# AmbiqAI/nnsp

Hardware: NVIDIA B200
Metric: audio-sec/sec (16 kHz streams, VAD+KWS+S2I cascade) (higher is better)
Workload: dtype int16 activations x int8 weights, int32/int64 accumulate (bit-exact integer path)

## Files before the change

### nnsp_b200/csrc/nnsp_engine.cu

```cuda
#include <cuda_runtime.h>
#include <mutex>
#include <new>
#include <stdlib.h>
#include <string.h>

#include "nnsp_feat.cuh"
#include "nnsp_host.h"
#include "nnsp_net.cuh"
#include "nnsp_tma.cuh"

namespace nnsp {

std::atomic<long long> g_launches{0}, g_tc5_launches{0};
std::atomic<long long> g_cascade_net_launches[3] = {};

static std::mutex g_mu;
static DevTables *g_dev_tables[64] = { nullptr };
static int g_sm_count[64] = { 0 };

int select_device(int device)
{
    int n = 0;
    cudaError_t e = cudaGetDeviceCount(&n);
    if (e != cudaSuccess || n <= 0) {
        nnsp_set_error("no CUDA device available (%s); nnsp-b200 has no CPU fallback", cudaGetErrorString(e));
        return NNSP_B200_ERR_CUDA;
    }
    if (device < 0 || device >= n || device >= 64) { nnsp_set_error("device %d out of range (have %d)", device, n); return NNSP_B200_ERR_ARG; }
    NNSP_CUDA(cudaSetDevice(device));
    std::lock_guard<std::mutex> lk(g_mu);
    if (!g_sm_count[device]) {
        cudaDeviceProp p;
        NNSP_CUDA(cudaGetDeviceProperties(&p, device));
        if (p.major < 10) {
            nnsp_set_error("device %d is sm_%d%d; this library is built for sm_100a only", device, p.major, p.minor);
            return NNSP_B200_ERR_CUDA;
        }
        g_sm_count[device] = p.multiProcessorCount;
    }
    return NNSP_B200_OK;
}
int sm_count(int device) { return g_sm_count[device] ? g_sm_count[device] : 148; }

static bool fill_dev_tables(const nnsp_tables *t, DevTables *d)
{
    bool ok = true;
    memset(d, 0, sizeof *d);
    for (int p = 0; p < 240; p++) d->win2[p] = make_int2((int)t->stft_win[2 * p], (int)t->stft_win[2 * p + 1]);
    auto unpack = [](int32_t w) { return make_int2((int)(int16_t)(w & 0xffff), (int)(w >> 16)); };
    for (int a = 0; a < 4; a++)
        for (int n = 0; n < 3; n++)
            for (int L = 0; L < 16; L++) d->tw0[a][n][L] = unpack(t->fft_tw[4 * (L + 16 * a) + 1 + n]);
    for (int n = 0; n < 3; n++)
        for (int L = 0; L < 16; L++) d->tw1[n][L] = unpack(t->fft_tw[16 * L + 1 + n]);
    for (int m = 0; m < 4; m++)
        for (int n = 0; n < 3; n++) d->tw2[m][n] = unpack(t->fft_tw[64 * m + 1 + n]);
    {
        auto one = [](int2 w) { return w.x == 0x7fff && w.y == 0; };
        auto diag = [](int2 w) { return w.x == w.y; };
        auto adiag = [](int2 w) { return w.y == -(w.x + 1); };
        if (!(one(d->tw2[0][0]) && one(d->tw2[0][1]) && one(d->tw2[0][2]) && adiag(d->tw2[1][0]) &&
              d->tw2[2][0].x == 0 && d->tw2[2][0].y == -32768 && adiag(d->tw2[2][1]) && diag(d->tw2[2][2]) && diag(d->tw2[3][0])))
            ok = false;
    }
    for (int k = 0; k < 256; k++) d->rtw[k] = unpack(t->rfft_tw[k]);
    d->rtw[256] = make_int2(0, 0);
    {
        int g = 0;
        for (int b = 0; b < 40; b++) {
            const int s0 = t->mel_start[b], e0 = t->mel_end[b], bin0 = s0 & ~3, ng = ((e0 | 3) - bin0 + 1) / 4;
            d->mel_meta[b] = (uint32_t)g | ((uint32_t)ng << 8) | ((uint32_t)bin0 << 16);
            if (ng > (b >= 24 ? MEL_MAXG0 : (b >= 8 ? MEL_MAXG1 : MEL_MAXG2)) || g + ng > MEL_GROUPS) ok = false;
            for (int i = 0; i < ng; i++, g++) {
                int w[4];
                for (int k = 0; k < 4; k++) {
                    const int bin = bin0 + 4 * i + k;
                    w[k] = (bin >= s0 && bin <= e0) ? (int)t->mel_taps[t->mel_off[b] + bin - s0] : 0;
                }
                if (g < MEL_GROUPS) d->mel_tap4[g] = make_int4(w[0], w[1], w[2], w[3]);
            }
        }
    }
    memcpy(d->log_lut, t->log_lut, sizeof d->log_lut);
    memcpy(d->tanh_lut, t->tanh_lut, sizeof d->tanh_lut);
    auto tanh_def = [&](int64_t xi) -> int64_t {
        if (xi >= (5 << 15)) return 0x7fff;
        int64_t kx = (xi - 512) >> 10;
        kx = kx < 0 ? 0 : kx;
        const int64_t v = (int64_t)t->tanh_lut[2 * kx] + (((xi - 512 - (kx << 10)) * (int64_t)t->tanh_lut[2 * kx + 1]) >> 15);
        return v > 0 ? v : 0;
    };
    for (int w = 0; w < 320; w++) {
        const int64_t k = w >= 1 ? (w - 1) >> 1 : 0, s = t->tanh_lut[2 * k + 1];
        int64_t lo = INT64_MIN, hi = INT64_MAX;
        for (int64_t dd = 0; dd < 512; dd++) {
            const int64_t y = tanh_def(512 * w + dd);
            lo = std::max(lo, y * 32768 - dd * s);
            hi = std::min(hi, (y + 1) * 32768 - dd * s);
        }
        if (lo >= hi || lo < 0 || lo + 511 * s > INT32_MAX) ok = false;
        d->tanh2[w] = make_int2((int)s, (int)lo);
    }
    d->tanh2[320] = make_int2(0, 0x7fff << 15);
    for (int64_t xi = 0; xi < (5 << 15) + 2048 && ok; xi++) {
        const int64_t w = std::min<int64_t>(xi >> 9, 320), dd = xi - (w << 9);
        if (((dd * d->tanh2[w].x + d->tanh2[w].y) >> 15) != tanh_def(xi)) ok = false;
    }
    return ok;
}

int get_device_tables(int device, const DevTables **out)
{
    std::lock_guard<std::mutex> lk(g_mu);
    if (!g_dev_tables[device]) {
        const nnsp_tables *t = nnsp_tables_get();
        if (!t) { nnsp_set_error("constant-table self check failed (fingerprint mismatch)"); return NNSP_B200_ERR_ARG; }
        DevTables h;
        if (!fill_dev_tables(t, &h)) { nnsp_set_error("constant tables do not have the structure the kernels compile in (mel group bounds, stage-2 twiddles, folded tanh table)"); return NNSP_B200_ERR_ARG; }
        DevTables *d = nullptr;
        NNSP_CUDA(cudaMalloc(&d, sizeof h));
        NNSP_CUDA(cudaMemcpy(d, &h, sizeof h, cudaMemcpyHostToDevice));
        NNSP_CUDA(cudaDeviceSynchronize());
        g_dev_tables[device] = d;
    }
    *out = g_dev_tables[device];
    return NNSP_B200_OK;
}

static void pack_matrix(uint32_t *dst, const int8_t *w, int nrows, int nrows_pad, int cols, int k4)
{
    for (int k = 0; k < k4; k++)
        for (int r = 0; r < nrows_pad; r++) {
            uint32_t word = 0;
            for (int b = 0; b < 4; b++) {
                const int c = 4 * k + b;
                const uint8_t v = (r < nrows && c < cols) ? (uint8_t)w[(size_t)r * cols + c] : 0;
                word |= (uint32_t)v << (8 * b);
            }
            dst[(size_t)k * nrows_pad + r] = word;
        }
}

int upload_model(const nnsp_b200_model *m, DeviceModel *out)
{
    DevModel &D = out->h;
    memset(&D, 0, sizeof D);
    D.nn_id = m->nn_id;
    D.numlayers = m->numlayers;
    D.n_out = m->size_layer[m->numlayers];
    D.feat_rshift = 30 - m->layer[0].qi;
    memcpy(D.mean, m->mean, sizeof D.mean);
    memcpy(D.stdR, m->stdR, sizeof D.stdR);
    for (int i = 0; i < 40; i++) {
        int64_t t = ((int64_t)-147963 - (int64_t)m->mean[i]) * (int64_t)m->stdR[i];
        t >>= D.feat_rshift;
        t = t > 32767 ? 32767 : (t < -32768 ? -32768 : t);
        D.silence[i] = (int16_t)t;
    }
    int woff = 0, boff = 0;
    for (int i = 0; i < m->numlayers; i++) {
        const nnsp_layer &L = m->layer[i];
        DevLayer &G = D.layer[i];
        G.type = L.type; G.act = L.act; G.rows = L.rows; G.cols = L.cols; G.acc32 = L.acc32;
        G.nrows = (L.type == NNSP_LAYER_LSTM) ? 4 * L.rows : L.rows;
        G.nrows_pad = (G.nrows + 31) & ~31;
        G.k4 = (L.cols + 3) / 4;
        G.k4rec = (L.type == NNSP_LAYER_LSTM) ? (L.rows + 3) / 4 : 0;
        const int qi_out = (L.type == NNSP_LAYER_LSTM) ? L.qi_next : L.qi;
        const int qs = (qi_out + L.qk) > 15 ? (qi_out + L.qk) : 15;
        G.sh_x = (L.type == NNSP_LAYER_LSTM) ? (L.qi_next - L.qi) : 0;
        G.sh_bias = qs - L.qb;
// ... 6 lines not shown
        if (L.cols > 480) { nnsp_set_error("layer %d: %d inputs exceed the exact-int32 dot-product bound (480)", i, L.cols); return NNSP_B200_ERR_UNSUPPORTED; }
    }
    if (D.h_stride > NNSP_B200_MAX_WIDTH) { nnsp_set_error("total LSTM state %d exceeds %d", D.h_stride, NNSP_B200_MAX_WIDTH); return NNSP_B200_ERR_UNSUPPORTED; }
    D.weight_words = (woff + 3) & ~3;
    D.bias_count = (boff + 7) & ~7;
    uint32_t *hw = (uint32_t *)calloc((size_t)D.weight_words + 4, 4);
    int16_t *hb = (int16_t *)calloc((size_t)D.bias_count + 8, 2);
    if (!hw || !hb) { free(hw); free(hb); return NNSP_B200_ERR_NOMEM; }
    for (int i = 0; i < m->numlayers; i++) {
        const nnsp_layer &L = m->layer[i];
        const DevLayer &G = D.layer[i];
        pack_matrix(hw + G.w_off, L.w, G.nrows, G.nrows_pad, L.cols, G.k4);
        if (L.type == NNSP_LAYER_LSTM) pack_matrix(hw + G.wrec_off, L.wrec, G.nrows, G.nrows_pad, L.rows, G.k4rec);
        memcpy(hb + G.bias_off, L.bias, (size_t)G.nrows * 2);
    }
    cudaError_t e1 = cudaMalloc(&out->wimg, (size_t)D.weight_words * 4);
    cudaError_t e2 = cudaMalloc(&out->bimg, (size_t)D.bias_count * 2);
    cudaError_t e3 = cudaMalloc(&out->d, sizeof D);
    if (e1 == cudaSuccess && e2 == cudaSuccess && e3 == cudaSuccess) {
        e1 = cudaMemcpy(out->wimg, hw, (size_t)D.weight_words * 4, cudaMemcpyHostToDevice);
        e2 = cudaMemcpy(out->bimg, hb, (size_t)D.bias_count * 2, cudaMemcpyHostToDevice);
        e3 = cudaMemcpy(out->d, &D, sizeof D, cudaMemcpyHostToDevice);
    }
    free(hw);
    free(hb);
    if (e1 != cudaSuccess || e2 != cudaSuccess || e3 != cudaSuccess) {
        nnsp_set_error("model upload failed: %s", cudaGetErrorString(e1 != cudaSuccess ? e1 : (e2 != cudaSuccess ? e2 : e3)));
        free_model(out);
        return NNSP_B200_ERR_CUDA;
    }
    return NNSP_B200_OK;
}

void free_model(DeviceModel *dm)
{
    if (dm->wimg) cudaFree(dm->wimg);
    if (dm->bimg) cudaFree(dm->bimg);
    if (dm->d) cudaFree(dm->d);
    dm->wimg = nullptr; dm->bimg = nullptr; dm->d = nullptr;
}

#ifndef FEAT_WARPS_PER_CTA
#define FEAT_WARPS_PER_CTA 8
#endif
constexpr int FEAT_WARPS = FEAT_WARPS_PER_CTA;
constexpr int FEAT_THREADS = FEAT_WARPS * 32;
#ifndef FEAT_CTAS_PER_SM
#define FEAT_CTAS_PER_SM 3
#endif
#ifndef FEAT_ITERS
#define FEAT_ITERS 8
#endif

struct FeatSmem {
    FeatSmemTables tb;
    FrameScratch fs[FEAT_WARPS * 2];
    int32_t norm[84];
};

template <bool RAGGED>
__global__ void __launch_bounds__(FEAT_THREADS, FEAT_CTAS_PER_SM)
feat_kernel(const DevTables *__restrict__ tables, const int16_t *__restrict__ pcm, long long stride,
            const int16_t *__restrict__ hist, int hist_frames, int s0, int ns, int T,
            int32_t *__restrict__ logmel, const int32_t *__restrict__ norm, int16_t *__restrict__ feat16,
            const int32_t *__restrict__ nfr)
{
    extern __shared__ __align__(128) unsigned char smem_raw[];
    FeatSmem &sm = *reinterpret_cast<FeatSmem *>(smem_raw);
    load_feat_tables(&sm.tb, tables, threadIdx.x, FEAT_THREADS);
    if (norm && threadIdx.x < 81) sm.norm[threadIdx.x] = norm[threadIdx.x];
    const int32_t *snorm = norm ? sm.norm : nullptr;
    __syncthreads();
    const int warp = threadIdx.x >> 5, lane = threadIdx.x & 31, half = lane >> 4, L = lane & 15;
    FrameScratch &fs = sm.fs[warp * 2 + half];
    const long long F = (long long)ns * T;
    const int hist_len = hist_frames * NNSP_B200_FRAME;
    for (long long f0 = ((long long)blockIdx.x * FEAT_WARPS + warp) * 2; f0 < F; f0 += (long long)gridDim.x * FEAT_WARPS * 2) {
        const long long f = f0 + half;
        bool valid = f < F;
        const long long fc = valid ? f : 0;
        const int s = s0 + (int)(fc / T), t = (int)(fc % T);
        if (RAGGED) {
            valid = valid && t < stream_frames(nfr, s, T);
            if (!__any_sync(0xffffffffu, valid)) continue;
        }
        const int base = (t - 2) * NNSP_B200_FRAME;
        const unsigned int *pw = reinterpret_cast<const unsigned int *>(pcm + (long long)s * stride + base) + L;
        const unsigned int *hw = reinterpret_cast<const unsigned int *>(hist + (long long)s * hist_len + hist_len + base) + L;
        const int pth = (2 - t) * (NNSP_B200_FRAME / 2);
        auto load_pair = [&](int a, int p) -> uint32_t {
            if (RAGGED && !valid) return 0u;
            return (p < pth) ? __ldg(hw + 16 * a) : __ldg(pw + 16 * a);
        };
        const long long row = ((long long)s * T + t) * NNSP_B200_NMEL;
        frame_logmel<false>(sm.tb, fs, L, load_pair, logmel + row, valid, FeatDump{}, snorm, feat16 + row);
    }
}

int launch_feature(const DevTables *tb, const FeatLaunch &a, int device, cudaStream_t st)
{
    static bool attr_set[64] = { false };
    static std::mutex attr_mu;
    std::unique_lock<std::mutex> attr_lk(attr_mu);
    if (!attr_set[device]) {
        NNSP_CUDA(cudaFuncSetAttribute(feat_kernel<false>, cudaFuncAttributeMaxDynamicSharedMemorySize, (int)sizeof(FeatSmem)));
        NNSP_CUDA(cudaFuncSetAttribute(feat_kernel<true>, cudaFuncAttributeMaxDynamicSharedMemorySize, (int)sizeof(FeatSmem)));
        attr_set[device] = true;
    }
    attr_lk.unlock();
    const long long F = (long long)a.ns * a.T;
    if (F <= 0) return NNSP_B200_OK;
    long long blocks = (F + FEAT_WARPS * 2 - 1) / (FEAT_WARPS * 2);
    const long long cap = (long long)sm_count(device) * FEAT_CTAS_PER_SM;
    long long iters = blocks / (cap * 8);
    iters = iters < FEAT_ITERS ? FEAT_ITERS : (iters > 4 * FEAT_ITERS ? 4 * FEAT_ITERS : iters);
    static const int iters_env = [] { const char *e = getenv("NNSP_B200_FEAT_ITERS"); return e ? atoi(e) : 0; }();
    if (iters_env > 0) iters = iters_env;
    const long long chunked = (blocks + iters - 1) / iters;
    if (blocks > cap) blocks = chunked > cap ? ((chunked + cap / 2) / cap) * cap : cap;
    static const int pad = [] { const char *e = getenv("NNSP_B200_FEAT_SMEM_PAD"); return e ? atoi(e) : 0; }();
    if (pad > 0) {
        static bool pad_set[64] = { false };
        if (!pad_set[device]) {
            NNSP_CUDA(cudaFuncSetAttribute(feat_kernel<false>, cudaFuncAttributeMaxDynamicSharedMemorySize, (int)sizeof(FeatSmem) + pad));
            NNSP_CUDA(cudaFuncSetAttribute(feat_kernel<true>, cudaFuncAttributeMaxDynamicSharedMemorySize, (int)sizeof(FeatSmem) + pad));
            pad_set[device] = true;
        }
    }
    const size_t smem = sizeof(FeatSmem) + (pad > 0 ? pad : 0);
    if (a.nfr)
        feat_kernel<true><<<(unsigned)blocks, FEAT_THREADS, smem, st>>>(tb, a.pcm, a.stride, a.hist, a.hist_frames, a.s0, a.ns, a.T,
                                                                       a.logmel, a.norm, a.feat16, a.nfr);
    else
        feat_kernel<false><<<(unsigned)blocks, FEAT_THREADS, smem, st>>>(tb, a.pcm, a.stride, a.hist, a.hist_frames, a.s0, a.ns, a.T,
                                                                        a.logmel, a.norm, a.feat16, nullptr);
    NNSP_LAUNCH_CHECK();
    return NNSP_B200_OK;
}

template <bool RAGGED>
__global__ void hist_kernel(const unsigned int *__restrict__ src, long long stride_words, unsigned int *__restrict__ hist,
                            int hist_frames, int wpf, int s0, int ns, int T_call, const int32_t *__restrict__ nfr)
{
    const int warp = (blockIdx.x * blockDim.x + threadIdx.x) >> 5, lane = threadIdx.x & 31;
    if (warp >= ns) return;
    const int s = s0 + warp;
    const int T = RAGGED ? stream_frames(nfr, s, T_call) : T_call;
    if (RAGGED && T == 0) return;
    const int words = hist_frames * wpf;
    const int keep = hist_frames - T;
// ... 203 lines not shown
        o.x = s0 | (s1 << 16); o.y = s2 | (s3 << 16); o.z = s4 | (s5 << 16); o.w = s6 | (s7 << 16);
        pcm[gidx] = o;
    }
}

int launch_ingest(const uint32_t *raw_dev, int16_t *pcm_dev, long long n_frames, int device, cudaStream_t st)
{
    if (n_frames <= 0) return NNSP_B200_OK;
    const long long groups = n_frames * (NNSP_B200_FRAME / 8);
    long long blocks = (groups + 255) / 256;
    const long long cap = (long long)sm_count(device) * 8;
    if (blocks > cap) blocks = cap;
    ingest_audadc_kernel<<<(unsigned)blocks, 256, 0, st>>>((const uint4 *)raw_dev, (uint4 *)pcm_dev, groups);
    NNSP_LAUNCH_CHECK();
    return NNSP_B200_OK;
}

__global__ void __launch_bounds__(256) int_peak_kernel(int *sink, int iters, int mode)
{
    int a[8], b[8];
    long long w[8];
#pragma unroll
    for (int i = 0; i < 8; i++) { a[i] = threadIdx.x * 7 + i * 13 + blockIdx.x; b[i] = a[i] ^ 0x55; w[i] = a[i]; }
    const int m = (int)threadIdx.x | 1, c = blockIdx.x + 3;
    if (mode == 0) {
        for (int it = 0; it < iters; it++) {
#pragma unroll
            for (int i = 0; i < 8; i++) { a[i] = a[i] * m + c; a[i] = a[i] * c + m; }
        }
    } else if (mode == 1) {
        for (int it = 0; it < iters; it++) {
#pragma unroll
            for (int i = 0; i < 8; i++) { a[i] = a[i] * m + c; b[i] = (b[i] >> 1) ^ it; }
#pragma unroll
            for (int i = 0; i < 8; i++) { a[i] = a[i] * c + m; b[i] = b[i] + (it | c); }
        }
    } else if (mode == 2) {
        for (int it = 0; it < iters; it++) {
#pragma unroll
            for (int i = 0; i < 8; i++) { w[i] += (long long)a[i] * m; w[i] += (long long)b[i] * c; }
        }
    } else {
        for (int it = 0; it < iters; it++) {
#pragma unroll
            for (int i = 0; i < 8; i++) { a[i] = __dp2a_lo(m, c, a[i]); a[i] = __dp2a_hi(c, m, a[i]); }
        }
    }
    int r = 0;
#pragma unroll
    for (int i = 0; i < 8; i++) r ^= a[i] ^ b[i] ^ (int)w[i] ^ (int)(w[i] >> 32);
    if (r == 0x7fffffff) sink[threadIdx.x] = r;
}

__global__ void __launch_bounds__(FEAT_THREADS)
feat_stages_kernel(const DevTables *__restrict__ tables, const int16_t *__restrict__ windows, int n,
                   int32_t *fft_in, int32_t *spec, int32_t *pspec, int32_t *mel, int32_t *logmel)
{
    extern __shared__ __align__(128) unsigned char smem_raw[];
    FeatSmem &sm = *reinterpret_cast<FeatSmem *>(smem_raw);
    load_feat_tables(&sm.tb, tables, threadIdx.x, FEAT_THREADS);
    __syncthreads();
    const int warp = threadIdx.x >> 5, lane = threadIdx.x & 31, half = lane >> 4, L = lane & 15;
    FrameScratch &fs = sm.fs[warp * 2 + half];
    for (int f0 = (blockIdx.x * FEAT_WARPS + warp) * 2; f0 < n; f0 += gridDim.x * FEAT_WARPS * 2) {
        const int f = f0 + half;
        const bool valid = f < n;
        const int fc = valid ? f : 0;
        const int16_t *w = windows + (long long)fc * 480;
        auto load_pair = [&](int a, int p) -> uint32_t { return *reinterpret_cast<const unsigned int *>(w + 2 * p); };
        FeatDump d;
        d.fft_in = fft_in ? fft_in + (long long)fc * 512 : nullptr;
        d.spec = spec ? spec + (long long)fc * 514 : nullptr;
        d.pspec = pspec ? pspec + (long long)fc * 257 : nullptr;
        d.mel = mel ? mel + (long long)fc * 40 : nullptr;
        frame_logmel<true>(sm.tb, fs, L, load_pair, logmel + (long long)fc * 40, valid, d);
    }
}

}

using namespace nnsp;

#define HOST_RING 4

struct nnsp_b200_batch {
    int device = 0, S = 0;
    cudaStream_t stream = nullptr;
    cudaStream_t xs[4] = { nullptr, nullptr, nullptr, nullptr };
    const DevTables *tables = nullptr;
    DeviceModel dm;
    MmaDeviceModel mm;
    bool mma_ok = false, split_ok = false;
    int nn_path = 0;
    int slides = 1;
    uint8_t *sp_planes[2] = { nullptr, nullptr };
    int32_t *sp_dec = nullptr;
    long long sp_cap_inf = 0;
    int16_t *feat16[2] = { nullptr, nullptr }; long long feat16_frames = 0;
    cudaStream_t nn_stream = nullptr;
    cudaEvent_t ev_feat[2] = { nullptr, nullptr }, ev_nn[2] = { nullptr, nullptr }, ev_nn0 = nullptr;
    bool nn_pending[2] = { false, false }, last_piped = false;
    unsigned pipe = 0;
    int32_t *norm_dev = nullptr;
    StreamState st{};
    int16_t thresh_prob = 0, th_count = 0;
    int32_t *logmel = nullptr; long long logmel_frames = 0;
    int16_t *d_pcm = nullptr; long long d_pcm_frames = 0;
    nnsp_b200_result *d_res = nullptr; long long d_res_frames = 0;
    NNSmemLayout lay{};
    int nn_ctas_per_sm = 1;
    cudaEvent_t ev[3] = { nullptr, nullptr, nullptr };
    bool ev_valid = false;
// ... 476 lines not shown
        NE_CUDA(cudaMemcpy(b->feat16[0], row5, N * 40 * sizeof(int16_t), cudaMemcpyHostToDevice));
        NE_CUDA(cudaDeviceSynchronize());
        NNLaunch l{};
        l.tables = b->tables; l.st = b->st; l.s0 = 0; l.ns = n; l.T = 1; l.taps = tp;
        l.thresh_prob = b->thresh_prob; l.th_count = b->th_count;
        if ((rc = launch_nn_split(b->mm, l, b->feat16[0], 0, 1, b->sp_planes[0], b->sp_planes[1], b->sp_dec, (int)b->sp_cap_inf, b->device, b->stream))) return done(rc);
    } else {
        NE_CUDA(cudaMemcpy(b->st.ctx, x, N * 240 * sizeof(int16_t), cudaMemcpyHostToDevice));
        NE_CUDA(cudaDeviceSynchronize());
        if (path == 2) {
            NNLaunch l{};
            l.tables = b->tables; l.st = b->st; l.s0 = 0; l.ns = n; l.T = 1; l.taps = tp; l.raw_ctx = 1;
            l.thresh_prob = b->thresh_prob; l.th_count = b->th_count;
            if ((rc = launch_nn_mma(b->mm, l, b->device, b->stream))) return done(rc);
        } else {
            NNArgs a{};
            a.model = b->dm.d; a.wimg = b->dm.wimg; a.bimg = b->dm.bimg; a.tables = b->tables; a.st = b->st;
            a.s0 = 0; a.ns = n; a.T = 1; a.taps = tp; a.raw_ctx = 1;
            a.thresh_prob = b->thresh_prob; a.th_count = b->th_count;
            int blocks = (n + NN_WARPS - 1) / NN_WARPS;
            const int cap = sm_count(b->device) * b->nn_ctas_per_sm;
            if (blocks > cap) blocks = cap;
            nn_kernel<<<blocks, NN_THREADS, b->lay.total, b->stream>>>(a, (int)b->lay.b, (int)b->lay.lut, (int)b->lay.model, (int)b->lay.scratch);
            g_launches.fetch_add(1);
            NE_CUDA(cudaGetLastError());
        }
    }
    NE_CUDA(cudaStreamSynchronize(b->stream));
    if (act && D.act_stride > 0) NE_CUDA(cudaMemcpy(act, t_act, N * D.act_stride * sizeof(int16_t), cudaMemcpyDeviceToHost));
    if (logits) NE_CUDA(cudaMemcpy(logits, t_logits, N * NO * sizeof(int32_t), cudaMemcpyDeviceToHost));
    if (h1 && HS > 0) NE_CUDA(cudaMemcpy(h1, t_h, N * HS * sizeof(int16_t), cudaMemcpyDeviceToHost));
    if (c1 && HS > 0) NE_CUDA(cudaMemcpy(c1, t_c, N * HS * sizeof(int32_t), cudaMemcpyDeviceToHost));
#undef NE_CUDA
    return done(NNSP_B200_OK);
}


int nnsp_b200_feature_stages(int device, const int16_t *windows, int n, int32_t *fft_in, int32_t *spec,
                             int32_t *pspec, int32_t *mel, int32_t *logmel)
{
    if (!windows || n <= 0) return NNSP_B200_ERR_ARG;
    int rc = select_device(device);
    if (rc) return rc;
    const DevTables *tb;
    if ((rc = get_device_tables(device, &tb))) return rc;
    int16_t *dw = nullptr;
    int32_t *dbuf = nullptr;
    const size_t per = 512 + 514 + 257 + 40 + 40;
    NNSP_CUDA(cudaMalloc(&dw, (size_t)n * 480 * 2));
    NNSP_CUDA(cudaMalloc(&dbuf, (size_t)n * per * 4));
    NNSP_CUDA(cudaMemcpy(dw, windows, (size_t)n * 480 * 2, cudaMemcpyHostToDevice));
    NNSP_CUDA(cudaDeviceSynchronize());
    int32_t *d_fi = dbuf, *d_sp = d_fi + (size_t)n * 512, *d_ps = d_sp + (size_t)n * 514, *d_me = d_ps + (size_t)n * 257, *d_lm = d_me + (size_t)n * 40;
    NNSP_CUDA(cudaFuncSetAttribute(feat_stages_kernel, cudaFuncAttributeMaxDynamicSharedMemorySize, (int)sizeof(FeatSmem)));
    int blocks = (n + FEAT_WARPS * 2 - 1) / (FEAT_WARPS * 2);
    if (blocks > 1024) blocks = 1024;
    feat_stages_kernel<<<blocks, FEAT_THREADS, sizeof(FeatSmem)>>>(tb, dw, n, d_fi, d_sp, d_ps, d_me, d_lm);
    NNSP_LAUNCH_CHECK();
    NNSP_CUDA(cudaDeviceSynchronize());
    if (fft_in) NNSP_CUDA(cudaMemcpy(fft_in, d_fi, (size_t)n * 512 * 4, cudaMemcpyDeviceToHost));
    if (spec) NNSP_CUDA(cudaMemcpy(spec, d_sp, (size_t)n * 514 * 4, cudaMemcpyDeviceToHost));
    if (pspec) NNSP_CUDA(cudaMemcpy(pspec, d_ps, (size_t)n * 257 * 4, cudaMemcpyDeviceToHost));
    if (mel) NNSP_CUDA(cudaMemcpy(mel, d_me, (size_t)n * 40 * 4, cudaMemcpyDeviceToHost));
    if (logmel) NNSP_CUDA(cudaMemcpy(logmel, d_lm, (size_t)n * 40 * 4, cudaMemcpyDeviceToHost));
    cudaFree(dw);
    cudaFree(dbuf);
    return NNSP_B200_OK;
}

int nnsp_b200_ingest_audadc(int device, const uint32_t *raw_dev, int16_t *pcm_dev, long long n_frames, void *stream)
{
    if (!raw_dev || !pcm_dev || n_frames < 0 || ((uintptr_t)raw_dev & 15) || ((uintptr_t)pcm_dev & 15)) {
        nnsp_set_error("ingest: null or not 16-byte aligned buffers");
        return NNSP_B200_ERR_ARG;
    }
    int rc = select_device(device);
    if (rc) return rc;
    return launch_ingest(raw_dev, pcm_dev, n_frames, device, (cudaStream_t)stream);
}

int nnsp_b200_table(const char *name, const void **data, int *elem_bytes)
{
    const nnsp_tables *t = nnsp_tables_get();
    if (!t || !name || !data || !elem_bytes) return NNSP_B200_ERR_ARG;
    struct { const char *n; const void *p; int eb, cnt; } tab[] = {
        { "stft_win", t->stft_win, 2, 480 }, { "fft_tw", t->fft_tw, 4, 256 }, { "rfft_tw", t->rfft_tw, 4, 256 },
        { "bitrev", t->bitrev, 2, 256 }, { "mel", t->mel, 2, 534 }, { "log_lut", t->log_lut, 2, 256 },
        { "tanh_lut", t->tanh_lut, 2, 384 },
    };
    for (auto &e : tab)
        if (!strcmp(e.n, name)) { *data = e.p; *elem_bytes = e.eb; return e.cnt; }
    return NNSP_B200_ERR_ARG;
}

int nnsp_b200_event_create(int device, void **event)
{
    int rc = select_device(device);
    if (rc) return rc;
    cudaEvent_t e;
    NNSP_CUDA(cudaEventCreate(&e));
    *event = (void *)e;
    return NNSP_B200_OK;
}
int nnsp_b200_event_record(void *event, void *stream) { NNSP_CUDA(cudaEventRecord((cudaEvent_t)event, (cudaStream_t)stream)); return NNSP_B200_OK; }
int nnsp_b200_event_elapsed_ms(void *start, void *stop, float *ms)
{
    NNSP_CUDA(cudaEventSynchronize((cudaEvent_t)stop));
    NNSP_CUDA(cudaEventElapsedTime(ms, (cudaEvent_t)start, (cudaEvent_t)stop));
    return NNSP_B200_OK;
}
// ... 59 lines not shown
```

### nnsp_b200/csrc/nnsp_engine.cuh

```cuda
#pragma once
#include <stdint.h>
#include "nnsp_b200.h"

namespace nnsp {

constexpr int MEL_GROUPS = 144;
constexpr int MEL_MAXG0 = 8, MEL_MAXG1 = 4, MEL_MAXG2 = 2;

struct DevTables {
    int4     mel_tap4[MEL_GROUPS];
    int2     win2[240];
    int2     tw0[4][3][16];
    int2     tw1[3][16];
    int2     tw2[4][3];
    int2     rtw[257];
    uint32_t mel_meta[40];
    int16_t  log_lut[256];
    int16_t  tanh_lut[384];
    int2     tanh2[321];
};

struct DevLayer {
    int type, act;
    int rows;
    int nrows;
    int nrows_pad;
    int cols, k4;
    int k4rec;
    int acc32;
    int sh_x;
    int sh_bias;
    int sh_out;
    int w_off, wrec_off;
    int bias_off;
};

struct DevModel {
    int      nn_id, numlayers;
    int      act_stride, h_stride, n_out;
    int      feat_rshift;
    int      weight_words, bias_count;
    int32_t  mean[40], stdR[40];
    int16_t  silence[40];
    DevLayer layer[NNSP_B200_MAX_LAYERS];
};

enum { SC_TRIGGER = 0, SC_OUT0 = 1, SC_CNT0 = 4, SC_ARGMAX_LAST = 12, SC_SLIDES = 13, SC_RAN = 14, SC_STAGE = 15, SC_N = 16 };

enum { CS_POS = 0, CS_CNT_KWS = 1, CS_CNT_S2I = 2, CS_AGE = 3, CS_N = 4 };

struct StreamState {
    int16_t *ctx;
    int16_t *h;
    int32_t *c;
    int16_t *scal;
    int16_t *hist;
    int32_t *lmhist;
    uint16_t *casc;
};

}
```

### nnsp_b200/csrc/nnsp_feat.cuh

```cuda
#pragma once
#include "nnsp_device.cuh"
#include "nnsp_engine.cuh"

namespace nnsp {

struct FeatSmemTables {
    int4     mel_tap4[MEL_GROUPS];
    int2     win2[240];
    int2     tw0[4][3][16];
    int2     tw1[3][16];
    int2     tw2[4][3];
    int2     rtw[257];
    uint32_t mel_meta[40];
    int16_t  log_lut[256];
};

struct alignas(16) FrameScratch {
    int2    x[272];
};

struct FeatDump {
    int32_t *fft_in, *spec, *pspec, *mel;
};

// ... 15 lines not shown
{
    const int32_t s1r = cr + dr, s1i = ci + di, d1r = cr - dr, d1i = ci - di;
    const int32_t o0r = add3(ar, br, s1r), o0i = add3(ai, bi, s1i);
    const int32_t o1r = add2sub(ar, br, s1r), o1i = add2sub(ai, bi, s1i);
    const int32_t o2r = sub2add(ar, br, d1i), o2i = sub3(ai, bi, d1r);
    const int32_t o3r = sub3(ar, br, d1i), o3i = sub2add(ai, bi, d1r);
    ar = mul_one_q15(o0r);
    ai = mul_one_q15(o0i);
    if (ALLONE) {
        cr = mul_one_q15(o1r); ci = mul_one_q15(o1i);
        br = mul_one_q15(o2r); bi = mul_one_q15(o2i);
        dr = mul_one_q15(o3r); di = mul_one_q15(o3i);
    } else {
        const int32_t w1r = w1.x, w1i = w1.y, w2r = w2.x, w2i = w2.y, w3r = w3.x, w3i = w3.y;
        cr = msub_q15(o1r, w1r, o1i, w1i); ci = madd_q15(o1r, w1i, o1i, w1r);
        br = msub_q15(o2r, w2r, o2i, w2i); bi = madd_q15(o2r, w2i, o2i, w2r);
        dr = msub_q15(o3r, w3r, o3i, w3i); di = madd_q15(o3r, w3i, o3i, w3r);
    }
}

enum { TW_ANY = 0, TW_ONE = 1, TW_NEGI = 2, TW_DIAG = 3, TW_ADIAG = 4 };
template <int KIND>
__device__ __forceinline__ void cmul_tw(int32_t or_, int32_t oi, int2 w, int32_t &re, int32_t &im)
{
    if (KIND == TW_ONE) { re = mul_one_q15(or_); im = mul_one_q15(oi); }
    else if (KIND == TW_NEGI) { re = oi; im = -or_; }
    else if (KIND == TW_DIAG) {
        re = (int32_t)(((int64_t)(or_ - oi) * (int64_t)w.x) >> 15);
        im = (int32_t)(((int64_t)(or_ + oi) * (int64_t)w.x) >> 15);
    } else if (KIND == TW_ADIAG) {
        re = (int32_t)(((int64_t)(or_ + oi) * (int64_t)w.x + (int64_t)oi) >> 15);
        im = (int32_t)(((int64_t)(oi - or_) * (int64_t)w.x - (int64_t)or_) >> 15);
    } else { re = msub_q15(or_, w.x, oi, w.y); im = madd_q15(or_, w.y, oi, w.x); }
}
template <int K1, int K2, int K3>
__device__ __forceinline__ void bfly4_tw(int32_t &ar, int32_t &ai, int32_t &cr, int32_t &ci,
                                         int32_t &br, int32_t &bi, int32_t &dr, int32_t &di,
                                         int2 w1, int2 w2, int2 w3)
{
    const int32_t s1r = cr + dr, s1i = ci + di, d1r = cr - dr, d1i = ci - di;
    const int32_t o0r = add3(ar, br, s1r), o0i = add3(ai, bi, s1i);
    const int32_t o1r = add2sub(ar, br, s1r), o1i = add2sub(ai, bi, s1i);
    const int32_t o2r = sub2add(ar, br, d1i), o2i = sub3(ai, bi, d1r);
    const int32_t o3r = sub3(ar, br, d1i), o3i = sub2add(ai, bi, d1r);
    ar = mul_one_q15(o0r);
    ai = mul_one_q15(o0i);
    cmul_tw<K1>(o1r, o1i, w1, cr, ci);
    cmul_tw<K2>(o2r, o2i, w2, br, bi);
    cmul_tw<K3>(o3r, o3i, w3, dr, di);
}

__device__ __forceinline__ int xpad(int p) { return p + (p >> 4); }

template <bool DUMP, typename LoadPair>
__device__ __forceinline__ void frame_logmel(const FeatSmemTables &tb, FrameScratch &fs, int L,
                                             LoadPair load_pair, int32_t *__restrict__ out_logmel,
                                             bool store, FeatDump dump, const int32_t *norm = nullptr,
                                             int16_t *__restrict__ out_feat = nullptr)
{
    int32_t xr[16], xi[16];
#pragma unroll
    for (int a = 0; a < 15; a++) {
        const int p = L + 16 * a;
        const uint32_t s = load_pair(a, p);
        const int2 w = tb.win2[p];
        xr[a] = (w.x * (int32_t)(int16_t)(s & 0xffff)) >> 15;
        xi[a] = (w.y * ((int32_t)s >> 16)) >> 15;
    }
    xr[15] = 0; xi[15] = 0;
    if (DUMP && dump.fft_in && store) {
#pragma unroll
        for (int a = 0; a < 16; a++) { dump.fft_in[2 * (L + 16 * a)] = xr[a]; dump.fft_in[2 * (L + 16 * a) + 1] = xi[a]; }
    }
#pragma unroll
    for (int a = 0; a < 4; a++) {
        bfly4<false>(xr[a], xi[a], xr[a + 4], xi[a + 4], xr[a + 8], xi[a + 8], xr[a + 12], xi[a + 12],
                     tb.tw0[a][0][L], tb.tw0[a][1][L], tb.tw0[a][2][L]);
    }
    {
        const int2 w1 = tb.tw1[0][L], w2 = tb.tw1[1][L], w3 = tb.tw1[2][L];
#pragma unroll
        for (int g = 0; g < 4; g++)
            bfly4<false>(xr[4 * g], xi[4 * g], xr[4 * g + 1], xi[4 * g + 1], xr[4 * g + 2], xi[4 * g + 2],
                         xr[4 * g + 3], xi[4 * g + 3], w1, w2, w3);
    }
#pragma unroll
    for (int a = 0; a < 16; a++) fs.x[xpad(L + 16 * a)] = make_int2(xr[a], xi[a]);
    __syncwarp();
#pragma unroll
    for (int b = 0; b < 16; b++) { const int2 v = fs.x[xpad(16 * L + b)]; xr[b] = v.x; xi[b] = v.y; }
    __syncwarp();
    bfly4_tw<TW_ONE, TW_ONE, TW_ONE>(xr[0], xi[0], xr[4], xi[4], xr[8], xi[8], xr[12], xi[12], tb.tw2[0][0], tb.tw2[0][1], tb.tw2[0][2]);
    bfly4_tw<TW_ADIAG, TW_ANY, TW_ANY>(xr[1], xi[1], xr[5], xi[5], xr[9], xi[9], xr[13], xi[13], tb.tw2[1][0], tb.tw2[1][1], tb.tw2[1][2]);
    bfly4_tw<TW_NEGI, TW_ADIAG, TW_DIAG>(xr[2], xi[2], xr[6], xi[6], xr[10], xi[10], xr[14], xi[14], tb.tw2[2][0], tb.tw2[2][1], tb.tw2[2][2]);
    bfly4_tw<TW_DIAG, TW_ANY, TW_ANY>(xr[3], xi[3], xr[7], xi[7], xr[11], xi[11], xr[15], xi[15], tb.tw2[3][0], tb.tw2[3][1], tb.tw2[3][2]);
#pragma unroll
    for (int g = 0; g < 4; g++)
        bfly4<true>(xr[4 * g], xi[4 * g], xr[4 * g + 1], xi[4 * g + 1], xr[4 * g + 2], xi[4 * g + 2],
                    xr[4 * g + 3], xi[4 * g + 3], make_int2(0, 0), make_int2(0, 0), make_int2(0, 0));
#pragma unroll
    for (int b = 0; b < 16; b++) {
        const int m = (int)(__brev((unsigned)(16 * L + b)) >> 24);
        fs.x[m] = make_int2(xr[b], xi[b]);
    }
    __syncwarp();
    int32_t pa[8], pb[8];
    int32_t p0 = 0, p256 = 0;
#pragma unroll
    for (int j = 0; j < 8; j++) {
        const bool centre = (j == 0 && L == 0);
        const int i = centre ? 128 : L + 16 * j;
        const int2 zi = fs.x[i], zr = fs.x[256 - i];
        const int2 w = tb.rtw[i], v = tb.rtw[256 - i];
        const int32_t er = (zi.x + zr.x) >> 1, ei = (zi.y - zr.y) >> 1;
        const int32_t orr = (zi.y + zr.y) >> 1, oi = (zr.x - zi.x) >> 1;
        const int32_t xr0 = er + msub_q15(orr, w.x, oi, w.y), xi0 = ei + madd_q15(orr, w.y, oi, w.x);
        pa[j] = (int32_t)(((int64_t)xr0 * xr0 + (int64_t)xi0 * xi0) >> 15);
        const int32_t fi = (zr.y - zi.y) >> 1, pi = (zi.x - zr.x) >> 1;
        const int32_t xr1 = er + msub_q15(orr, v.x, pi, v.y), xi1 = fi + madd_q15(orr, v.y, pi, v.x);
        pb[j] = (int32_t)(((int64_t)xr1 * xr1 + (int64_t)xi1 * xi1) >> 15);
        if (DUMP && dump.spec && store) {
            dump.spec[2 * i] = xr0; dump.spec[2 * i + 1] = xi0;
            if (!centre) { dump.spec[2 * (256 - i)] = xr1; dump.spec[2 * (256 - i) + 1] = xi1; }
        }
    }
    if (DUMP && L == 0) {
        const int2 z0 = fs.x[0], w = tb.rtw[0];
        const int32_t er = z0.x, orr = z0.y;
        const int32_t xr0 = er + msub_q15(orr, w.x, 0, w.y), xi0 = madd_q15(orr, w.y, 0, w.x);
        const int32_t re = z0.x - z0.y;
        p0 = (int32_t)(((int64_t)xr0 * xr0 + (int64_t)xi0 * xi0) >> 15);
        p256 = (int32_t)(((int64_t)re * re) >> 15);
        if (dump.spec && store) { dump.spec[0] = xr0; dump.spec[1] = xi0; dump.spec[512] = re; dump.spec[513] = 0; }
    }
    __syncwarp();
    int32_t *ps = reinterpret_cast<int32_t *>(fs.x);
#pragma unroll
    for (int j = 0; j < 8; j++) {
        const bool centre = (j == 0 && L == 0);
        const int i = centre ? 128 : L + 16 * j;
        ps[i] = pa[j];
        if (!centre) ps[256 - i] = pb[j];
    }
    if (DUMP && L == 0) { ps[0] = p0; ps[256] = p256; }
    __syncwarp();
    if (DUMP && dump.pspec && store)
        for (int i = L; i < 257; i += 16) dump.pspec[i] = ps[i];
#pragma unroll
    for (int r = 0; r < 3; r++) {
        const int b = 39 - L - 16 * r;
        if (b >= 0) {
            const uint32_t meta = tb.mel_meta[b];
            const int ng = (meta >> 8) & 0xff;
            const int4 *tap = &tb.mel_tap4[meta & 0xff];
            const int4 *bin = reinterpret_cast<const int4 *>(&ps[meta >> 16]);
            int64_t m0 = 0, m1 = 0;
#pragma unroll
            for (int i = 0; i < (r == 0 ? MEL_MAXG0 : (r == 1 ? MEL_MAXG1 : MEL_MAXG2)); i++) {
                if (i < ng) {
                    const int4 w = tap[i], v = bin[i];
                    m0 += (int64_t)w.x * (int64_t)v.x; m1 += (int64_t)w.y * (int64_t)v.y;
                    m0 += (int64_t)w.z * (int64_t)v.z; m1 += (int64_t)w.w * (int64_t)v.w;
                }
            }
            const int32_t mel = sat32_dev((m0 + m1) >> 15);
            if (DUMP && dump.mel && store) dump.mel[b] = mel;
            if (store) {
                const int32_t lm = log10_q15(mel, tb.log_lut);
                if (norm) out_feat[b] = standardise(lm, norm[b], norm[40 + b], norm[80]);
                else out_logmel[b] = lm;
            }
        }
    }
    __syncwarp();
}

}
```

Baseline: 5.271 million.

## Compute mel filterbank with u8 IMMA tensor-core tiles over byte-plane power spectra

```diff
diff --git a/nnsp_b200/csrc/nnsp_engine.cu b/nnsp_b200/csrc/nnsp_engine.cu
--- a/nnsp_b200/csrc/nnsp_engine.cu
+++ b/nnsp_b200/csrc/nnsp_engine.cu
@@ -6,6 +6,7 @@
 
 #include "nnsp_feat.cuh"
 #include "nnsp_host.h"
+#include "nnsp_mma.cuh"
 #include "nnsp_net.cuh"
 #include "nnsp_tma.cuh"
 
@@ -81,6 +82,48 @@
             }
         }
     }
+    {
+        auto tap = [&](int b, int bin) -> int {
+            return (bin >= t->mel_start[b] && bin <= t->mel_end[b]) ? (int)t->mel_taps[t->mel_off[b] + bin - t->mel_start[b]] : 0;
+        };
+        int blk = 0;
+        for (int j = 0; j < MEL_NTILES; j++) {
+            int lo = 256, hi = -1;
+            for (int b = 8 * j; b < 8 * j + 8; b++) { lo = std::min(lo, (int)t->mel_start[b]); hi = std::max(hi, (int)t->mel_end[b]); }
+            const int ks0 = lo / 32, nk = hi < lo ? 0 : hi / 32 - ks0 + 1;
+            if (lo < 0 || hi > 255 || blk + nk > MEL_BLOCKS) { ok = false; break; }
+            d->mel_tile[j] = (uint32_t)ks0 | ((uint32_t)nk << 8) | ((uint32_t)blk << 16);
+            for (int k = 0; k < nk; k++, blk++)
+                for (int l = 0; l < 32; l++) {
+                    uint32_t v[4] = { 0, 0, 0, 0 };
+                    for (int c = 0; c < 8; c++) {
+                        const int x = tap(8 * j + (l >> 2), 32 * (ks0 + k) + 16 * (c >> 2) + 4 * (l & 3) + (c & 3));
+                        v[c >> 2] |= (uint32_t)(x & 0xff) << (8 * (c & 3));
+                        v[2 + (c >> 2)] |= (uint32_t)((x >> 8) & 0xff) << (8 * (c & 3));
+                    }
+                    d->mel_frag[blk][l] = make_uint4(v[0], v[1], v[2], v[3]);
+                }
+        }
+        for (int b = 0; b < 40 && ok; b++) {
+            const uint32_t m = d->mel_tile[b >> 3];
+            const int ks0 = m & 0xff, nk = (m >> 8) & 0xff, blk0 = m >> 16, g = b & 7;
+            for (int bin = 0; bin <= 256; bin++) {
+                int x = 0;
+                const int k = bin / 32 - ks0, r = bin % 32;
+                if (k >= 0 && k < nk) {
+                    const uint4 f = d->mel_frag[blk0 + k][4 * g + ((r & 15) >> 2)];
+                    const uint32_t lo8 = r < 16 ? f.x : f.y, hi8 = r < 16 ? f.z : f.w;
+                    x = (int)((lo8 >> (8 * (r & 3))) & 0xff) + 256 * (int)((hi8 >> (8 * (r & 3))) & 0xff);
+                }
+                if (x != tap(b, bin)) ok = false;
+            }
+        }
+    }
+    for (int k = 0; k < 8; k++)
+        for (int L = 0; L < 16; L++) {
+            const int i = 8 * L + 1 + k;
+            d->rtw8[k][L] = make_int4(d->rtw[i].x, d->rtw[i].y, d->rtw[256 - i].x, d->rtw[256 - i].y);
+        }
     memcpy(d->log_lut, t->log_lut, sizeof d->log_lut);
     memcpy(d->tanh_lut, t->tanh_lut, sizeof d->tanh_lut);
     auto tanh_def = [&](int64_t xi) -> int64_t {
@@ -116,7 +159,7 @@
         const nnsp_tables *t = nnsp_tables_get();
         if (!t) { nnsp_set_error("constant-table self check failed (fingerprint mismatch)"); return NNSP_B200_ERR_ARG; }
         DevTables h;
-        if (!fill_dev_tables(t, &h)) { nnsp_set_error("constant tables do not have the structure the kernels compile in (mel group bounds, stage-2 twiddles, folded tanh table)"); return NNSP_B200_ERR_ARG; }
+        if (!fill_dev_tables(t, &h)) { nnsp_set_error("constant tables do not have the structure the kernels compile in (mel group bounds, mel MMA blocks, stage-2 twiddles, folded tanh table)"); return NNSP_B200_ERR_ARG; }
         DevTables *d = nullptr;
         NNSP_CUDA(cudaMalloc(&d, sizeof h));
         NNSP_CUDA(cudaMemcpy(d, &h, sizeof h, cudaMemcpyHostToDevice));
@@ -229,6 +272,134 @@
 #define FEAT_ITERS 8
 #endif
 
+#ifndef NNSP_FEAT_MEL_MMA
+#define NNSP_FEAT_MEL_MMA 1
+#endif
+
+#if NNSP_FEAT_MEL_MMA
+constexpr int FS_X_ODD = 1024, FS_P_ODD = 2176, FS_PITCH = 3216;
+static_assert(FS_P_ODD == FS_X_ODD + (int)sizeof(FrameScratch) - 1024 && FS_X_ODD >= 1024 && FS_PITCH >= FS_P_ODD + 1024 &&
+              FS_PITCH % 32 == 16, "slot layout");
+static_assert(FEAT_WARPS * 2 == 16 && MEL_NTILES <= FEAT_WARPS, "a round is the 16 rows of one m16n8k32 tile");
+struct alignas(16) FeatSlot { unsigned char b[FS_PITCH]; };
+
+struct FeatSmem {
+    FeatSmemTables tb;
+    uint4    mel_frag[MEL_BLOCKS][32];
+    int4     rtw8[8][16];
+    uint32_t mel_tile[MEL_NTILES];
+    int32_t  norm[84];
+    long long row[2][16];
+    FeatSlot fs[16];
+};
+
+__device__ __forceinline__ void imma_u8u8(uint32_t (&c)[4], const uint32_t (&a)[4], uint32_t b0, uint32_t b1)
+{
+    asm volatile("mma.sync.aligned.m16n8k32.row.col.s32.u8.u8.s32 {%0,%1,%2,%3}, {%4,%5,%6,%7}, {%8,%9}, {%0,%1,%2,%3};"
+                 : "+r"(c[0]), "+r"(c[1]), "+r"(c[2]), "+r"(c[3])
+                 : "r"(a[0]), "r"(a[1]), "r"(a[2]), "r"(a[3]), "r"(b0), "r"(b1));
+}
+
+__device__ __forceinline__ int32_t mel_from_classes(uint32_t a0, uint32_t a8, uint32_t a16, uint32_t a24, uint32_t a32)
+{
+    const uint32_t u1 = a8 + (a0 >> 8), u2 = a16 + (u1 >> 8), u3 = a24 + (u2 >> 8);
+    const uint32_t hi = (a32 << 8) + u3;
+    const bool sat = a32 >= (1u << 14) || hi >= (1u << 22);
+    return sat ? 0x7fffffff : (int32_t)((hi << 9) | ((u2 & 0xff) << 1) | ((u1 >> 7) & 1));
+}
+
+__device__ __forceinline__ void feat_mel_tile(const FeatSmem &sm, int j, int lane, int par, int32_t *__restrict__ logmel,
+                                              const int32_t *norm, int16_t *__restrict__ feat16)
+{
+    const uint32_t meta = sm.mel_tile[j];
+    const int ks0 = meta & 0xff, nk = (meta >> 8) & 0xff;
+    const uint4 *frag = &sm.mel_frag[meta >> 16][lane];
+    uint32_t addr = ldm_lane_addr(sm.fs[0].b + (par ? FS_P_ODD : 0), FS_PITCH, lane) + 32 * ks0;
+    uint32_t acc[5][4] = {};
+#pragma unroll 1
+    for (int k = 0; k < nk; k++, addr += 32, frag += 32) {
+        uint32_t p0[4], p1[4], p2[4], p3[4];
+        load_a_ldm(addr, p0);
+        load_a_ldm(addr + 256, p1);
+        load_a_ldm(addr + 512, p2);
+        load_a_ldm(addr + 768, p3);
+        const uint4 t = *frag;
+        imma_u8u8(acc[0], p0, t.x, t.y);
+        imma_u8u8(acc[1], p1, t.x, t.y);
+        imma_u8u8(acc[2], p2, t.x, t.y);
+        imma_u8u8(acc[3], p3, t.x, t.y);
+        imma_u8u8(acc[4], p3, t.z, t.w);
+        imma_u8u8(acc[1], p0, t.z, t.w);
+        imma_u8u8(acc[2], p1, t.z, t.w);
+        imma_u8u8(acc[3], p2, t.z, t.w);
+    }
+    const int g = lane >> 2, b = 8 * j + 2 * (lane & 3);
+#pragma unroll
+    for (int h = 0; h < 2; h++) {
+        const long long row = sm.row[par][g + 8 * h];
+        if (row < 0) continue;
+        int32_t lm[2];
+#pragma unroll
+        for (int c = 0; c < 2; c++) {
+            const int e = 2 * h + c;
+            lm[c] = log10_q15(mel_from_classes(acc[0][e], acc[1][e], acc[2][e], acc[3][e], acc[4][e]), sm.tb.log_lut);
+        }
+        if (norm) {
+            const uint32_t y0 = (uint16_t)standardise(lm[0], norm[b], norm[40 + b], norm[80]);
+            const uint32_t y1 = (uint16_t)standardise(lm[1], norm[b + 1], norm[41 + b], norm[80]);
+            *reinterpret_cast<uint32_t *>(feat16 + row + b) = y0 | (y1 << 16);
+        } else {
+            *reinterpret_cast<int2 *>(logmel + row + b) = make_int2(lm[0], lm[1]);
+        }
+    }
+}
+
+template <bool RAGGED>
+__global__ void __launch_bounds__(FEAT_THREADS, FEAT_CTAS_PER_SM)
+feat_kernel(const DevTables *__restrict__ tables, const int16_t *__restrict__ pcm, long long stride,
+            const int16_t *__restrict__ hist, int hist_frames, int s0, int ns, int T,
+            int32_t *__restrict__ logmel, const int32_t *__restrict__ norm, int16_t *__restrict__ feat16,
+            const int32_t *__restrict__ nfr)
+{
+    extern __shared__ __align__(128) unsigned char smem_raw[];
+    FeatSmem &sm = *reinterpret_cast<FeatSmem *>(smem_raw);
+    load_feat_tables(&sm.tb, tables, threadIdx.x, FEAT_THREADS);
+    for (int i = threadIdx.x; i < MEL_BLOCKS * 32; i += FEAT_THREADS) (&sm.mel_frag[0][0])[i] = (&tables->mel_frag[0][0])[i];
+    if (threadIdx.x < 8 * 16) (&sm.rtw8[0][0])[threadIdx.x] = (&tables->rtw8[0][0])[threadIdx.x];
+    if (threadIdx.x < MEL_NTILES) sm.mel_tile[threadIdx.x] = tables->mel_tile[threadIdx.x];
+    if (norm && threadIdx.x < 81) sm.norm[threadIdx.x] = norm[threadIdx.x];
+    const int32_t *snorm = norm ? sm.norm : nullptr;
+    __syncthreads();
+    const int warp = threadIdx.x >> 5, lane = threadIdx.x & 31, half = lane >> 4, L = lane & 15, r = warp * 2 + half;
+    unsigned char *slot = sm.fs[r].b;
+    const long long F = (long long)ns * T;
+    const int hist_len = hist_frames * NNSP_B200_FRAME;
+    int par = 0;
+    for (long long f0 = (long long)blockIdx.x * 16; f0 < F; f0 += (long long)gridDim.x * 16, par ^= 1) {
+        const long long f = f0 + r;
+        bool valid = f < F;
+        const long long fc = valid ? f : 0;
+        const int s = s0 + (int)(fc / T), t = (int)(fc % T);
+        if (RAGGED) valid = valid && t < stream_frames(nfr, s, T);
+        if (!RAGGED || __any_sync(0xffffffffu, valid)) {
+            const int base = (t - 2) * NNSP_B200_FRAME;
+            const unsigned int *pw = reinterpret_cast<const unsigned int *>(pcm + (long long)s * stride + base) + L;
+            const unsigned int *hw = reinterpret_cast<const unsigned int *>(hist + (long long)s * hist_len + hist_len + base) + L;
+            const int pth = (2 - t) * (NNSP_B200_FRAME / 2);
+            auto load_pair = [&](int a, int p) -> uint32_t {
+                if (RAGGED && !valid) return 0u;
+                return (p < pth) ? __ldg(hw + 16 * a) : __ldg(pw + 16 * a);
+            };
+            int2 *x = reinterpret_cast<int2 *>(slot + (par ? FS_X_ODD : 0));
+            frame_fft<false, true>(sm.tb, x, L, load_pair, false, FeatDump{});
+            pspec_planes(&sm.rtw8[0][0], x, slot + (par ? FS_P_ODD : 0), L);
+        }
+        if (L == 0) sm.row[par][r] = valid ? ((long long)s * T + t) * NNSP_B200_NMEL : -1;
+        __syncthreads();
+        if (warp < MEL_NTILES) feat_mel_tile(sm, warp, lane, par, logmel, snorm, feat16);
+    }
+}
+#else
 struct FeatSmem {
     FeatSmemTables tb;
     FrameScratch fs[FEAT_WARPS * 2];
@@ -273,6 +444,7 @@
         frame_logmel<false>(sm.tb, fs, L, load_pair, logmel + row, valid, FeatDump{}, snorm, feat16 + row);
     }
 }
+#endif
 
 int launch_feature(const DevTables *tb, const FeatLaunch &a, int device, cudaStream_t st)
 {
@@ -582,12 +754,16 @@
     if (r == 0x7fffffff) sink[threadIdx.x] = r;
 }
 
+struct FeatStagesSmem {
+    FeatSmemTables tb;
+    FrameScratch fs[FEAT_WARPS * 2];
+};
 __global__ void __launch_bounds__(FEAT_THREADS)
 feat_stages_kernel(const DevTables *__restrict__ tables, const int16_t *__restrict__ windows, int n,
                    int32_t *fft_in, int32_t *spec, int32_t *pspec, int32_t *mel, int32_t *logmel)
 {
     extern __shared__ __align__(128) unsigned char smem_raw[];
-    FeatSmem &sm = *reinterpret_cast<FeatSmem *>(smem_raw);
+    FeatStagesSmem &sm = *reinterpret_cast<FeatStagesSmem *>(smem_raw);
     load_feat_tables(&sm.tb, tables, threadIdx.x, FEAT_THREADS);
     __syncthreads();
     const int warp = threadIdx.x >> 5, lane = threadIdx.x & 31, half = lane >> 4, L = lane & 15;
@@ -1170,10 +1346,10 @@
     NNSP_CUDA(cudaMemcpy(dw, windows, (size_t)n * 480 * 2, cudaMemcpyHostToDevice));
     NNSP_CUDA(cudaDeviceSynchronize());
     int32_t *d_fi = dbuf, *d_sp = d_fi + (size_t)n * 512, *d_ps = d_sp + (size_t)n * 514, *d_me = d_ps + (size_t)n * 257, *d_lm = d_me + (size_t)n * 40;
-    NNSP_CUDA(cudaFuncSetAttribute(feat_stages_kernel, cudaFuncAttributeMaxDynamicSharedMemorySize, (int)sizeof(FeatSmem)));
+    NNSP_CUDA(cudaFuncSetAttribute(feat_stages_kernel, cudaFuncAttributeMaxDynamicSharedMemorySize, (int)sizeof(FeatStagesSmem)));
     int blocks = (n + FEAT_WARPS * 2 - 1) / (FEAT_WARPS * 2);
     if (blocks > 1024) blocks = 1024;
-    feat_stages_kernel<<<blocks, FEAT_THREADS, sizeof(FeatSmem)>>>(tb, dw, n, d_fi, d_sp, d_ps, d_me, d_lm);
+    feat_stages_kernel<<<blocks, FEAT_THREADS, sizeof(FeatStagesSmem)>>>(tb, dw, n, d_fi, d_sp, d_ps, d_me, d_lm);
     NNSP_LAUNCH_CHECK();
     NNSP_CUDA(cudaDeviceSynchronize());
     if (fft_in) NNSP_CUDA(cudaMemcpy(fft_in, d_fi, (size_t)n * 512 * 4, cudaMemcpyDeviceToHost));
diff --git a/nnsp_b200/csrc/nnsp_engine.cuh b/nnsp_b200/csrc/nnsp_engine.cuh
--- a/nnsp_b200/csrc/nnsp_engine.cuh
+++ b/nnsp_b200/csrc/nnsp_engine.cuh
@@ -6,6 +6,7 @@
 
 constexpr int MEL_GROUPS = 144;
 constexpr int MEL_MAXG0 = 8, MEL_MAXG1 = 4, MEL_MAXG2 = 2;
+constexpr int MEL_NTILES = 5, MEL_BLOCKS = 12;
 
 struct DevTables {
     int4     mel_tap4[MEL_GROUPS];
@@ -18,6 +19,9 @@
     int16_t  log_lut[256];
     int16_t  tanh_lut[384];
     int2     tanh2[321];
+    uint4    mel_frag[MEL_BLOCKS][32];
+    uint32_t mel_tile[MEL_NTILES];
+    int4     rtw8[8][16];
 };
 
 struct DevLayer {
diff --git a/nnsp_b200/csrc/nnsp_feat.cuh b/nnsp_b200/csrc/nnsp_feat.cuh
--- a/nnsp_b200/csrc/nnsp_feat.cuh
+++ b/nnsp_b200/csrc/nnsp_feat.cuh
@@ -91,11 +91,8 @@
 
 __device__ __forceinline__ int xpad(int p) { return p + (p >> 4); }
 
-template <bool DUMP, typename LoadPair>
-__device__ __forceinline__ void frame_logmel(const FeatSmemTables &tb, FrameScratch &fs, int L,
-                                             LoadPair load_pair, int32_t *__restrict__ out_logmel,
-                                             bool store, FeatDump dump, const int32_t *norm = nullptr,
-                                             int16_t *__restrict__ out_feat = nullptr)
+template <bool DUMP, bool ZPAD, typename LoadPair>
+__device__ __forceinline__ void frame_fft(const FeatSmemTables &tb, int2 *x, int L, LoadPair load_pair, bool store, FeatDump dump)
 {
     int32_t xr[16], xi[16];
 #pragma unroll
@@ -124,10 +121,10 @@
                          xr[4 * g + 3], xi[4 * g + 3], w1, w2, w3);
     }
 #pragma unroll
-    for (int a = 0; a < 16; a++) fs.x[xpad(L + 16 * a)] = make_int2(xr[a], xi[a]);
-    __syncwarp();
-#pragma unroll
-    for (int b = 0; b < 16; b++) { const int2 v = fs.x[xpad(16 * L + b)]; xr[b] = v.x; xi[b] = v.y; }
+    for (int a = 0; a < 16; a++) x[xpad(L + 16 * a)] = make_int2(xr[a], xi[a]);
+    __syncwarp();
+#pragma unroll
+    for (int b = 0; b < 16; b++) { const int2 v = x[xpad(16 * L + b)]; xr[b] = v.x; xi[b] = v.y; }
     __syncwarp();
     bfly4_tw<TW_ONE, TW_ONE, TW_ONE>(xr[0], xi[0], xr[4], xi[4], xr[8], xi[8], xr[12], xi[12], tb.tw2[0][0], tb.tw2[0][1], tb.tw2[0][2]);
     bfly4_tw<TW_ADIAG, TW_ANY, TW_ANY>(xr[1], xi[1], xr[5], xi[5], xr[9], xi[9], xr[13], xi[13], tb.tw2[1][0], tb.tw2[1][1], tb.tw2[1][2]);
@@ -140,9 +137,18 @@
 #pragma unroll
     for (int b = 0; b < 16; b++) {
         const int m = (int)(__brev((unsigned)(16 * L + b)) >> 24);
-        fs.x[m] = make_int2(xr[b], xi[b]);
-    }
-    __syncwarp();
+        x[ZPAD ? xpad(m) : m] = make_int2(xr[b], xi[b]);
+    }
+    __syncwarp();
+}
+
+template <bool DUMP, typename LoadPair>
+__device__ __forceinline__ void frame_logmel(const FeatSmemTables &tb, FrameScratch &fs, int L,
+                                             LoadPair load_pair, int32_t *__restrict__ out_logmel,
+                                             bool store, FeatDump dump, const int32_t *norm = nullptr,
+                                             int16_t *__restrict__ out_feat = nullptr)
+{
+    frame_fft<DUMP, false>(tb, fs.x, L, load_pair, store, dump);
     int32_t pa[8], pb[8];
     int32_t p0 = 0, p256 = 0;
 #pragma unroll
@@ -214,4 +220,44 @@
     __syncwarp();
 }
 
-}
+__device__ __forceinline__ void byte_planes4(uint32_t v0, uint32_t v1, uint32_t v2, uint32_t v3, uint32_t (&w)[4])
+{
+    const uint32_t t0 = __byte_perm(v0, v1, 0x5140), t1 = __byte_perm(v0, v1, 0x7362);
+    const uint32_t t2 = __byte_perm(v2, v3, 0x5140), t3 = __byte_perm(v2, v3, 0x7362);
+    w[0] = __byte_perm(t0, t2, 0x5410); w[1] = __byte_perm(t0, t2, 0x7632);
+    w[2] = __byte_perm(t1, t3, 0x5410); w[3] = __byte_perm(t1, t3, 0x7632);
+}
+
+__device__ __forceinline__ void store_planes8(uint8_t *dst, const uint32_t (&v)[8])
+{
+    uint32_t lo[4], hi[4];
+    byte_planes4(v[0], v[1], v[2], v[3], lo);
+    byte_planes4(v[4], v[5], v[6], v[7], hi);
+#pragma unroll
+    for (int q = 0; q < 4; q++) *reinterpret_cast<uint2 *>(dst + 256 * q) = make_uint2(lo[q], hi[q]);
+}
+
+__device__ __forceinline__ void pspec_planes(const int4 *rtw8, const int2 *x, uint8_t *planes, int L)
+{
+    uint32_t pa[8], pb[8];
+#pragma unroll
+    for (int k = 0; k < 8; k++) {
+        const int i = 8 * L + 1 + k;
+        const int2 zi = x[xpad(i)], zr = x[xpad(256 - i)];
+        const int4 w = rtw8[16 * k + L];
+        const int32_t er = (zi.x + zr.x) >> 1, ei = (zi.y - zr.y) >> 1;
+        const int32_t orr = (zi.y + zr.y) >> 1, oi = (zr.x - zi.x) >> 1;
+        const int32_t xr0 = er + msub_q15(orr, w.x, oi, w.y), xi0 = ei + madd_q15(orr, w.y, oi, w.x);
+        pa[k] = (uint32_t)(((int64_t)xr0 * xr0 + (int64_t)xi0 * xi0) >> 15);
+        const int32_t fi = (zr.y - zi.y) >> 1, pi = (zi.x - zr.x) >> 1;
+        const int32_t xr1 = er + msub_q15(orr, w.z, pi, w.w), xi1 = fi + madd_q15(orr, w.w, pi, w.z);
+        pb[k] = (uint32_t)(((int64_t)xr1 * xr1 + (int64_t)xi1 * xi1) >> 15);
+    }
+    uint32_t b8 = __shfl_up_sync(0xffffffffu, pa[7], 1, 16);
+    if (L == 0) b8 = 0;
+    __syncwarp();
+    store_planes8(planes + 8 * L, { b8, pa[0], pa[1], pa[2], pa[3], pa[4], pa[5], pa[6] });
+    store_planes8(planes + 248 - 8 * L, { pb[7], pb[6], pb[5], pb[4], pb[3], pb[2], pb[1], pb[0] });
+}
+
+}
```

Result: faster. 5.325 million, median of 6 (+1.0%).
